# facebookresearch/metamorph

Measured on AMD Instinct MI355X. Metric: train tokens/sec (LLaMA-3-8B + SigLIP-SO400M, seq2048, 256 img toks), whole job, higher is better.
Workload: dtype bf16

## Files before the change

metamorph_amd/build.py:

```python
from __future__ import annotations

import hashlib
import os
import subprocess
import sys

PKG = os.path.dirname(os.path.abspath(__file__))
CSRC = os.path.join(PKG, "csrc")
LIBDIR = os.path.join(PKG, "lib")
LIB = os.path.join(LIBDIR, "libmm355.so")
SOURCES = ["gemm_bf16.hip", "rowwise.hip", "elementwise.hip", "attn.hip", "attn2.hip", "attn4.hip", "attn4_bwd.hip", "decode.hip", "decode_w8.hip", "decode_w4.hip", "decode_kv8.hip", "attn_extend.hip", "gemm_w8.hip", "gemm_w4.hip", "losses.hip", "linear_ce.hip"]
HEADERS = ["mm355_common.h", "gemm_common.h", "splitk.h", "decode_wq.h", "attn2.h", "rowsum.h"] + sorted(
    os.path.join(d, f) for d in ("attn4_gen", "attn4_bwd_gen")
    for f in os.listdir(os.path.join(CSRC, d)) if f.endswith(".inc"))
BASE_FLAGS = ["--offload-arch=gfx950", "-O3", "-std=c++17", "-fPIC", "-Wno-unused-result"]
FLAGS = BASE_FLAGS + ["-mllvm", "-amdgpu-mfma-vgpr-form=1"]
FLAGS_OF = {f: BASE_FLAGS + ["-mllvm", "-amdgpu-spill-vgpr-to-agpr=0"] for f in ("attn4.hip", "attn4_bwd.hip")}


def _hipcc():
    for c in (os.environ.get("HIPCC"), "/opt/rocm/bin/hipcc", "hipcc"):
        if c and (os.path.isabs(c) and os.path.exists(c) or not os.path.isabs(c)):
            return c
    raise RuntimeError("hipcc not found")


def _digest():
    h = hashlib.sha256()
    for f in SOURCES + HEADERS:
        h.update(open(os.path.join(CSRC, f), "rb").read())
    h.update(open(os.path.join(os.path.dirname(PKG), "include", "mm355.h"), "rb").read())
    h.update(" ".join(FLAGS).encode())
    h.update(repr(sorted(FLAGS_OF.items())).encode())
    return h.hexdigest()


def build(force: bool = False, verbose: bool = True) -> str:
    os.makedirs(LIBDIR, exist_ok=True)
    stamp = os.path.join(LIBDIR, "libmm355.stamp")
    dig = _digest()
    if not force and os.path.exists(LIB) and os.path.exists(stamp) and open(stamp).read().strip() == dig:
        return LIB
    hipcc = _hipcc()
    objs = []
    procs = []
    for src in SOURCES:
        obj = os.path.join(LIBDIR, src.replace(".hip", ".o"))
        cmd = [hipcc, *FLAGS_OF.get(src, FLAGS), "-c", os.path.join(CSRC, src), "-o", obj]
        if verbose:
            print("[mm355 build]", " ".join(cmd), flush=True)
        procs.append((src, subprocess.Popen(cmd, stdout=subprocess.PIPE, stderr=subprocess.STDOUT)))
        objs.append(obj)
    for src, p in procs:
        out, _ = p.communicate()
        if p.returncode != 0:
            raise RuntimeError(f"hipcc failed on {src}:\n{out.decode(errors='replace')}")
    cmd = [hipcc, "--offload-arch=gfx950", "-shared", "-fPIC", "-o", LIB, *objs]
    if verbose:
        print("[mm355 build]", " ".join(cmd), flush=True)
    subprocess.check_call(cmd)
    with open(stamp, "w") as f:
        f.write(dig)
    return LIB


# ... 3 lines not shown
```

metamorph_amd/csrc/elementwise.hip:

```cpp
#include "mm355_common.h"
#include <algorithm>

namespace {

constexpr int NT = 256;
constexpr int MAX_GRID = 256 * 16;

inline unsigned grid_for(int64_t work_items) {
    int64_t g = (work_items + NT - 1) / NT;
    if (g > MAX_GRID) g = MAX_GRID;
    if (g < 1) g = 1;
    return (unsigned)g;
}

__global__ void rope_table_kernel(uint16_t* __restrict__ cos_o, uint16_t* __restrict__ sin_o, int L, int d, float theta) {
    const int half = d >> 1;
    for (int64_t i = blockIdx.x * (int64_t)NT + threadIdx.x; i < (int64_t)L * half; i += (int64_t)gridDim.x * NT) {
        const int l = (int)(i / half), j = (int)(i % half);
        const float inv = 1.0f / powf(theta, (float)(2 * j) / (float)d);
        const float ang = (float)l * inv;
        const uint16_t c = f2bf(cosf(ang)), s = f2bf(sinf(ang));
        cos_o[(int64_t)l * d + j] = c; cos_o[(int64_t)l * d + half + j] = c;
        sin_o[(int64_t)l * d + j] = s; sin_o[(int64_t)l * d + half + j] = s;
    }
// ... 125 lines not shown
        float f[8];
        unpack8(*(const u32x4*)(x + i), f);
#pragma unroll
        for (int e = 0; e < 8; ++e) f[e] = kind == MM355_GELU_ERF ? gelu_erf_f(f[e]) : gelu_tanh_f(f[e]);
        *(u32x4*)(y + i) = pack8(f);
    }
}
__global__ __launch_bounds__(NT) void gelu_bwd_kernel(const uint16_t* __restrict__ x, const uint16_t* __restrict__ dy, uint16_t* __restrict__ dx, int64_t n, int kind) {
    for (int64_t i = (blockIdx.x * (int64_t)NT + threadIdx.x) * 8; i < n; i += (int64_t)gridDim.x * NT * 8) {
        float f[8], g[8];
        unpack8(*(const u32x4*)(x + i), f);
        unpack8(*(const u32x4*)(dy + i), g);
#pragma unroll
        for (int e = 0; e < 8; ++e) g[e] *= kind == MM355_GELU_ERF ? gelu_erf_grad(f[e]) : gelu_tanh_grad(f[e]);
        *(u32x4*)(dx + i) = pack8(g);
    }
}

__global__ __launch_bounds__(NT) void scale_kernel(uint16_t* __restrict__ x, int64_t n, const float* __restrict__ s_dev, float s_host) {
    const float s = (s_dev ? *s_dev : 1.0f) * s_host;
    const int64_t nv = n >> 3;
    for (int64_t v = blockIdx.x * (int64_t)NT + threadIdx.x; v < nv; v += (int64_t)gridDim.x * NT) {
        float f[8];
        unpack8(*(const u32x4*)(x + v * 8), f);
#pragma unroll
        for (int e = 0; e < 8; ++e) f[e] *= s;
        *(u32x4*)(x + v * 8) = pack8(f);
    }
    if (blockIdx.x == 0 && threadIdx.x < (n & 7)) { const int64_t i = (nv << 3) + threadIdx.x; x[i] = f2bf(bf2f(x[i]) * s); }
}
template <typename TX>
__global__ __launch_bounds__(NT) void axpy_kernel(uint16_t* __restrict__ y, const TX* __restrict__ x, int64_t n, const float* __restrict__ s_dev,
                                                  float s_host, int accumulate) {
    const float s = (s_dev ? *s_dev : 1.0f) * s_host;
    for (int64_t i = blockIdx.x * (int64_t)NT + threadIdx.x; i < n; i += (int64_t)gridDim.x * NT) {
        float xv;
        if constexpr (sizeof(TX) == 2) xv = bf2f(x[i]); else xv = x[i];
        float r = s * xv;
        if (accumulate) r += bf2f(y[i]);
        y[i] = f2bf(r);
    }
}
__global__ __launch_bounds__(NT) void cast2d_kernel(const float* __restrict__ in, int64_t ld_in, uint16_t* __restrict__ out, int64_t ld_out, int64_t rows, int cols) {
    const int cv = cols >> 3;
    const int64_t total = rows * cv;
    for (int64_t i = blockIdx.x * (int64_t)NT + threadIdx.x; i < total; i += (int64_t)gridDim.x * NT) {
        const int64_t r = i / cv; const int c = (int)(i % cv) * 8;
        const f32x4 a = *(const f32x4*)(in + r * ld_in + c), b = *(const f32x4*)(in + r * ld_in + c + 4);
        const float f[8] = {a.x, a.y, a.z, a.w, b.x, b.y, b.z, b.w};
        *(u32x4*)(out + r * ld_out + c) = pack8(f);
    }
}

__global__ __launch_bounds__(NT) void adamw_kernel(float* __restrict__ p32, float* __restrict__ m, float* __restrict__ v, const uint16_t* __restrict__ g,
                                                   uint16_t* __restrict__ pout, int64_t n, float lr, float b1, float b2, float eps, float wd,
                                                   float bc1, float bc2, const float* __restrict__ gs_dev) {
    const float gs = gs_dev ? *gs_dev : 1.0f;
    const float inv_sqrt_bc2 = rsqrtf(bc2);
    const float step = lr / bc1;
    for (int64_t i = blockIdx.x * (int64_t)NT + threadIdx.x; i < n; i += (int64_t)gridDim.x * NT) {
        const float gr = bf2f(g[i]) * gs;
        float p = p32[i] * (1.0f - lr * wd);
        const float mi = m[i] * b1 + (1.0f - b1) * gr;
        const float vi = v[i] * b2 + (1.0f - b2) * gr * gr;
        const float denom = sqrtf(vi) * inv_sqrt_bc2 + eps;
        p -= step * (mi / denom);
        m[i] = mi; v[i] = vi; p32[i] = p;
        pout[i] = f2bf(p);
    }
}
__global__ __launch_bounds__(NT) void sumsq_kernel(const uint16_t* __restrict__ x, int64_t n, float* __restrict__ partials) {
    __shared__ float red[NT / 64];
    float s = 0.f;
    const int64_t nv = n >> 3;
    for (int64_t v = blockIdx.x * (int64_t)NT + threadIdx.x; v < nv; v += (int64_t)gridDim.x * NT) {
        float f[8];
        unpack8(*(const u32x4*)(x + v * 8), f);
#pragma unroll
        for (int e = 0; e < 8; ++e) s += f[e] * f[e];
    }
    if (blockIdx.x == 0 && threadIdx.x < (n & 7)) { const float f = bf2f(x[(nv << 3) + threadIdx.x]); s += f * f; }
    s = block_sum<NT>(s, red);
    if (threadIdx.x == 0) partials[blockIdx.x] = s;
}
__global__ __launch_bounds__(NT) void sumsq_finish_kernel(const float* __restrict__ partials, int count, float* __restrict__ out) {
    __shared__ float red[NT / 64];
    float s = 0.f;
    for (int i = threadIdx.x; i < count; i += NT) s += partials[i];
    s = block_sum<NT>(s, red);
    if (threadIdx.x == 0) out[0] += s;
}
__global__ void clip_coef_kernel(const float* __restrict__ sumsq, float max_norm, float pre, float* __restrict__ coef) {
    const float nrm = sqrtf(*sumsq);
    float c = max_norm > 0.f ? max_norm / (nrm + 1e-6f) : 1.0f;
    if (c > 1.0f) c = 1.0f;
    *coef = c * pre;
}

template <typename TI>
__global__ __launch_bounds__(NT) void im2col_kernel(const TI* __restrict__ img, int N, int H, int W, int p, uint16_t* __restrict__ out, int Kp) {
    const int gh = H / p, gw = W / p, kreal = 3 * p * p;
    const int64_t total = (int64_t)N * gh * gw * Kp;
    for (int64_t i = blockIdx.x * (int64_t)NT + threadIdx.x; i < total; i += (int64_t)gridDim.x * NT) {
        const int k = (int)(i % Kp);
        const int64_t pr = i / Kp;
        uint16_t val = 0;
        if (k < kreal) {
            const int c = k / (p * p), dy = (k / p) % p, dx = k % p;
            const int px = (int)(pr % gw), py = (int)((pr / gw) % gh); const int64_t n = pr / ((int64_t)gw * gh);
            const TI x = img[((n * 3 + c) * H + (int64_t)py * p + dy) * W + (int64_t)px * p + dx];
            if constexpr (sizeof(TI) == 2) val = x; else val = f2bf(x);
        }
        out[i] = val;
    }
}

__global__ __launch_bounds__(NT) void splice_gather_kernel(const uint16_t* __restrict__ embed, const uint16_t* __restrict__ proj, const int32_t* __restrict__ src,
                                                           uint16_t* __restrict__ out, int64_t rows, int h) {
    const int64_t row = blockIdx.x * (int64_t)(NT / 64) + (threadIdx.x >> 6);
// ... 103 lines not shown
    if (!gu || !dact || !dgu || M <= 0 || I <= 0 || (I & 7)) return MM355_EINVAL;
    LAUNCH(swiglu_bwd_kernel, grid_for(M * (I / 8)), gu, dact, dgu, act, M, (int)I);
}
extern "C" int mm355_swiglu_bwd_t(const mm355_bf16* gu, const mm355_bf16* dact, mm355_bf16* dgu, mm355_bf16* actT, mm355_bf16* dguT,
                                  int64_t M, int64_t I, void* stream) {
    (void)hipGetLastError();
    if (!gu || !dact || !dgu || !actT || !dguT || M <= 0 || I <= 0) return MM355_EINVAL;
    if ((M & 63) || (I & 63)) return MM355_EUNSUPPORTED;
    if (M / 64 > 65535) return MM355_EINVAL;
    hipLaunchKernelGGL(swiglu_bwd_t_kernel, dim3((unsigned)(I / 64), (unsigned)(M / 64)), dim3(256), 0, (hipStream_t)stream, gu, dact, dgu,
                       actT, dguT, M, (int)I);
    return mm_launch_status();
}
extern "C" int mm355_gelu_fwd(const mm355_bf16* x, mm355_bf16* y, int64_t n, int kind, void* stream) {
    (void)hipGetLastError();
    if (!x || !y || n <= 0 || (n & 7)) return MM355_EINVAL;
    LAUNCH(gelu_fwd_kernel, grid_for(n / 8), x, y, n, kind);
}
extern "C" int mm355_gelu_bwd(const mm355_bf16* x, const mm355_bf16* dy, mm355_bf16* dx, int64_t n, int kind, void* stream) {
    (void)hipGetLastError();
    if (!x || !dy || !dx || n <= 0 || (n & 7)) return MM355_EINVAL;
    LAUNCH(gelu_bwd_kernel, grid_for(n / 8), x, dy, dx, n, kind);
}
extern "C" int mm355_scale_bf16(mm355_bf16* x, int64_t n, const float* s_dev, float s_host, void* stream) {
    (void)hipGetLastError();
    if (!x || n <= 0 || !mm_aligned16(x)) return MM355_EINVAL;
    LAUNCH(scale_kernel, grid_for(n / 8 + 1), x, n, s_dev, s_host);
}
extern "C" int mm355_axpy_bf16(mm355_bf16* y, const mm355_bf16* x, int64_t n, const float* s_dev, float s_host, int accumulate, void* stream) {
    (void)hipGetLastError();
    if (!x || !y || n <= 0) return MM355_EINVAL;
    LAUNCH(axpy_kernel<uint16_t>, grid_for(n), y, x, n, s_dev, s_host, accumulate);
}
extern "C" int mm355_axpy_f32_to_bf16(mm355_bf16* y, const float* x, int64_t n, float s_host, int accumulate, void* stream) {
    (void)hipGetLastError();
    if (!x || !y || n <= 0) return MM355_EINVAL;
    LAUNCH(axpy_kernel<float>, grid_for(n), y, x, n, (const float*)nullptr, s_host, accumulate);
}
extern "C" int mm355_axpy_f32_to_bf16_dev(mm355_bf16* y, const float* x, int64_t n, const float* s_dev, float s_host, int accumulate, void* stream) {
    (void)hipGetLastError();
    if (!x || !y || n <= 0) return MM355_EINVAL;
    LAUNCH(axpy_kernel<float>, grid_for(n), y, x, n, s_dev, s_host, accumulate);
}
extern "C" int mm355_cast_f32_bf16_2d(const float* in, int64_t ld_in, mm355_bf16* out, int64_t ld_out, int64_t rows, int64_t cols, void* stream) {
    (void)hipGetLastError();
    if (!in || !out || rows <= 0 || cols <= 0 || (cols & 7) || (ld_in & 3) || (ld_out & 7)) return MM355_EINVAL;
    LAUNCH(cast2d_kernel, grid_for(rows * (cols / 8)), in, ld_in, out, ld_out, rows, (int)cols);
}
extern "C" int mm355_adamw_shard(float* p32, float* m, float* v, const mm355_bf16* g, mm355_bf16* p_out, int64_t n, float lr, float beta1,
                                 float beta2, float eps, float weight_decay, float bias_corr1, float bias_corr2, const float* grad_scale_dev,
                                 void* stream) {
    (void)hipGetLastError();
    if (!p32 || !m || !v || !g || !p_out || n <= 0 || bias_corr1 <= 0.f || bias_corr2 <= 0.f) return MM355_EINVAL;
    LAUNCH(adamw_kernel, grid_for(n), p32, m, v, g, p_out, n, lr, beta1, beta2, eps, weight_decay, bias_corr1, bias_corr2, grad_scale_dev);
}
extern "C" int mm355_sumsq_bf16(const mm355_bf16* x, int64_t n, float* out, float* partials, void* stream) {
    (void)hipGetLastError();
    if (!x || !out || !partials || n <= 0 || !mm_aligned16(x)) return MM355_EINVAL;
    const int blocks = (int)std::min<int64_t>((n / 8 + NT) / NT, MM355_SUMSQ_PARTIALS);
    hipLaunchKernelGGL(sumsq_kernel, dim3(blocks), dim3(NT), 0, (hipStream_t)stream, x, n, partials);
    hipLaunchKernelGGL(sumsq_finish_kernel, dim3(1), dim3(NT), 0, (hipStream_t)stream, (const float*)partials, blocks, out);
    return mm_launch_status();
}
extern "C" int mm355_clip_coef(const float* sumsq, float max_norm, float pre_scale, float* coef, void* stream) {
    (void)hipGetLastError();
    if (!sumsq || !coef) return MM355_EINVAL;
    hipLaunchKernelGGL(clip_coef_kernel, dim3(1), dim3(1), 0, (hipStream_t)stream, sumsq, max_norm, pre_scale, coef);
    return mm_launch_status();
}
extern "C" int mm355_im2col_patch(const void* images, int images_are_f32, int64_t N, int64_t H, int64_t W, int64_t p, mm355_bf16* out, int64_t Kp,
                                  void* stream) {
    (void)hipGetLastError();
    if (!images || !out || N <= 0 || H < p || W < p || p <= 0 || Kp < 3 * p * p) return MM355_EINVAL;
    const int64_t total = N * (H / p) * (W / p) * Kp;
    if (images_are_f32) LAUNCH(im2col_kernel<float>, grid_for(total), (const float*)images, (int)N, (int)H, (int)W, (int)p, out, (int)Kp);
    LAUNCH(im2col_kernel<uint16_t>, grid_for(total), (const uint16_t*)images, (int)N, (int)H, (int)W, (int)p, out, (int)Kp);
}
extern "C" int mm355_splice_gather(const mm355_bf16* embed, const mm355_bf16* proj, const int32_t* src, mm355_bf16* out, int64_t rows, int64_t h,
                                   void* stream) {
    (void)hipGetLastError();
    if (!embed || !src || !out || rows <= 0 || h <= 0 || (h & 7)) return MM355_EINVAL;
    LAUNCH(splice_gather_kernel, (unsigned)((rows + 3) / 4), embed, proj, src, out, rows, (int)h);
}
extern "C" int mm355_rows_gather(const mm355_bf16* in, int64_t ld_in, const int32_t* idx, mm355_bf16* out, int64_t ld_out, int64_t R, int64_t h,
                                 void* stream) {
    (void)hipGetLastError();
    if (!in || !idx || !out || R <= 0 || h <= 0 || (h & 7) || (ld_in & 7) || (ld_out & 7)) return MM355_EINVAL;
    LAUNCH(rows_gather_kernel, (unsigned)((R + 3) / 4), in, ld_in, idx, out, ld_out, R, (int)h);
}
extern "C" int mm355_rows_scatter_add(const mm355_bf16* src, int64_t ld_src, const int32_t* idx, mm355_bf16* dst, int64_t ld_dst, int64_t R,
                                      int64_t h, void* stream) {
    (void)hipGetLastError();
    if (!src || !idx || !dst || R <= 0 || h <= 0 || (h & 7) || (ld_src & 7) || (ld_dst & 7)) return MM355_EINVAL;
    LAUNCH(rows_scatter_add_kernel, (unsigned)((R + 3) / 4), src, ld_src, idx, dst, ld_dst, R, (int)h);
}
extern "C" int mm355_embed_grad(const mm355_bf16* dout, const int32_t* tok, const int32_t* seg_start, const int32_t* pos, int64_t n_seg,
                                mm355_bf16* dembed, int64_t h, int accumulate, void* stream) {
    (void)hipGetLastError();
    if (!dout || !tok || !seg_start || !pos || !dembed || n_seg <= 0 || h <= 0 || (h & 7)) return MM355_EINVAL;
    LAUNCH(embed_grad_kernel, (unsigned)((n_seg + 3) / 4), dout, tok, seg_start, pos, n_seg, dembed, (int)h, accumulate);
}
```

metamorph_amd/csrc/gemm_bf16.hip:

```cpp
#include "gemm_common.h"
#include "splitk.h"
#include <type_traits>
#include <cstdlib>

namespace {

MM_DEV void gemm_epilogue_swiglu(f32x4 (&acc)[8][4], const GemmArgs& a, unsigned char* smem, int m0, int tn, int wm, int wn, int wave, int lane) {
    constexpr int TN = 64;
    const int fr = lane & 15, fq = lane >> 4;
    const int M = a.M, I = (int)a.res_mod;
    float* stg = (float*)smem + wave * (16 * TN);
    const int row_l = lane >> 2, k4 = lane & 3;
    uint16_t* gu = (uint16_t*)a.C;
    uint16_t* act = (uint16_t*)a.res;
    const int ch0 = tn * 128 + wn * 32;
#pragma unroll
    for (int i = 0; i < 8; ++i) {
        __builtin_amdgcn_fence(__ATOMIC_RELEASE, "wavefront");
        __builtin_amdgcn_wave_barrier();
#pragma unroll
        for (int j = 0; j < 4; ++j)
#pragma unroll
            for (int r = 0; r < 4; ++r) stg[(fq * 4 + r) * TN + j * 16 + fr] = acc[i][j][r];
        __builtin_amdgcn_fence(__ATOMIC_RELEASE, "wavefront");
        __builtin_amdgcn_wave_barrier();
        const int grow = m0 + wm * 128 + i * 16 + row_l;
        if (grow < M) {
            float g[8], u[8], o[8];
            const f32x4 g0 = *(const f32x4*)(stg + row_l * TN + k4 * 8), g1 = *(const f32x4*)(stg + row_l * TN + k4 * 8 + 4);
            const f32x4 u0 = *(const f32x4*)(stg + row_l * TN + 32 + k4 * 8), u1 = *(const f32x4*)(stg + row_l * TN + 32 + k4 * 8 + 4);
            g[0] = g0.x; g[1] = g0.y; g[2] = g0.z; g[3] = g0.w; g[4] = g1.x; g[5] = g1.y; g[6] = g1.z; g[7] = g1.w;
            u[0] = u0.x; u[1] = u0.y; u[2] = u0.z; u[3] = u0.w; u[4] = u1.x; u[5] = u1.y; u[6] = u1.z; u[7] = u1.w;
            const u32x4 gp = pack8(g), up = pack8(u);
            const int ch = ch0 + k4 * 8;
            *(u32x4*)(gu + (int64_t)grow * a.ldc + ch) = gp;
            *(u32x4*)(gu + (int64_t)grow * a.ldc + I + ch) = up;
            float gb[8], ub[8];
            unpack8(gp, gb);
            unpack8(up, ub);
#pragma unroll
            for (int e = 0; e < 8; ++e) o[e] = round_bf(gb[e] / (1.0f + __expf(-gb[e]))) * ub[e];
            *(u32x4*)(act + (int64_t)grow * a.ldr + ch) = pack8(o);
        }
    }
}

constexpr int SWB_TROW = 144;
constexpr int SWB_T = 3 * 32 * SWB_TROW;
constexpr int SWB_LDS = 32768 + 8 * SWB_T;
MM_DEV void gemm_epilogue_swiglu_bwd(f32x4 (&acc)[8][4], const GemmArgs& a, unsigned char* smem, int m0, int n0, int wm, int wn, int wave, int lane) {
    constexpr int TN = 64, PF = 4;
    typedef __attribute__((ext_vector_type(4))) short s16x4;
    typedef __attribute__((address_space(3))) s16x4* lds4_t;
    const int fr = lane & 15, fq = lane >> 4;
// ... 640 lines not shown
    return (int64_t)a.ntm * a.ntn;
}

template <int ABL = 0>
int launch_gemm_pp_t(GemmArgs a, hipStream_t s) {
    static std::atomic<uint64_t> lds_ok{0};
    if (mm_ensure_dynamic_lds((const void*)gemm_pp_kernel<ABL>, PP_LDS, lds_ok) != MM355_OK) return MM355_ELAUNCH;
    const int64_t total = pp_prepare(a);
    if (total <= 0 || total > 0x7fffffff) return MM355_EINVAL;
#ifdef MM355_PP_PERSIST
    hipLaunchKernelGGL((gemm_pp_kernel<ABL>), dim3((unsigned)std::min<int64_t>(total, MM355_PP_PERSIST)), dim3(512), PP_LDS, s, a);
#else
    hipLaunchKernelGGL((gemm_pp_kernel<ABL>), dim3((unsigned)total), dim3(512), PP_LDS, s, a);
#endif
    return mm_launch_status();
}

int launch_gemm_pp_pair(GemmArgs a0, GemmArgs a1, hipStream_t s) {
    static std::atomic<uint64_t> lds_ok{0};
    if (mm_ensure_dynamic_lds((const void*)gemm_pp_pair_kernel, PP_LDS, lds_ok) != MM355_OK) return MM355_ELAUNCH;
    const int64_t n0 = pp_prepare(a0), n1 = pp_prepare(a1);
    if (n0 <= 0 || n1 <= 0 || n0 + n1 > 0x7fffffff) return MM355_EINVAL;
    hipLaunchKernelGGL(gemm_pp_pair_kernel, dim3((unsigned)(n0 + n1)), dim3(512), PP_LDS, s, a0, a1, (int)n0);
    return mm_launch_status();
}

bool pp_eligible(const GemmArgs& a) {
    if (a.K < 128 || (a.K & 127)) return false;
    const int64_t ea = (256 * a.lda + a.K) * 2;
    const int64_t eb = (256 * a.ldb + a.K) * 2;
    return ea < 0x7fffffffLL && eb < 0x7fffffffLL;
}

int launch_gemm_pp(GemmArgs a, hipStream_t s) {
    if (!pp_eligible(a)) return launch_gemm<256, 256, 2, 4, true, 1>(a, s);
    return launch_gemm_pp_t(a, s);
}

template <int BM, int BN, int WM, int WN, bool GLDS, int PIPE = 0>
int launch_gemm(GemmArgs a, hipStream_t s) {
    constexpr int STAGE = (BM + BN) * 128;
    constexpr int LDS = 2 * STAGE;
    auto kern = gemm_nt_kernel<BM, BN, WM, WN, GLDS, PIPE>;
    static std::atomic<uint64_t> lds_ok{0};
    if (mm_ensure_dynamic_lds((const void*)kern, LDS, lds_ok) != MM355_OK) return MM355_ELAUNCH;
    a.ntm = (a.M + BM - 1) / BM;
    a.ntn = (a.N + BN - 1) / BN;
    const int64_t total = (int64_t)a.ntm * a.ntn;
    if (total <= 0 || total > 0x7fffffff) return MM355_EINVAL;
    hipLaunchKernelGGL(kern, dim3((unsigned)total), dim3(WM * WN * 64), LDS, s, a);
    return mm_launch_status();
}

__global__ __launch_bounds__(256) void transpose_kernel(const uint16_t* __restrict__ in, int64_t ld_in, int rows, int cols,
                                                        uint16_t* __restrict__ out, int64_t ld_out) {
    __shared__ uint16_t tile[64][64 + 2];
    const int r0 = blockIdx.y * 64, c0 = blockIdx.x * 64;
    const int tid = threadIdx.x;
#pragma unroll
    for (int i = 0; i < 2; ++i) {
        const int v = tid + i * 256, r = v >> 3, c = (v & 7) * 8;
        const int gr = r0 + r, gc = c0 + c;
        uint16_t tmp[8];
        if (gr < rows && gc + 8 <= cols) {
            *(u32x4*)tmp = *(const u32x4*)(in + (int64_t)gr * ld_in + gc);
        } else {
#pragma unroll
            for (int e = 0; e < 8; ++e) tmp[e] = (gr < rows && gc + e < cols) ? in[(int64_t)gr * ld_in + gc + e] : (uint16_t)0;
        }
#pragma unroll
        for (int e = 0; e < 8; ++e) tile[r][c + e] = tmp[e];
    }
    __syncthreads();
#pragma unroll
    for (int i = 0; i < 2; ++i) {
        const int v = tid + i * 256, c = v >> 3, r = (v & 7) * 8;
        const int gc = c0 + c, gr = r0 + r;
        if (gc >= cols) continue;
        uint16_t tmp[8];
#pragma unroll
        for (int e = 0; e < 8; ++e) tmp[e] = tile[r + e][c];
        if (gr + 8 <= rows && ((ld_out & 7) == 0)) {
            *(u32x4*)(out + (int64_t)gc * ld_out + gr) = *(const u32x4*)tmp;
        } else {
            for (int e = 0; e < 8; ++e)
                if (gr + e < rows) out[(int64_t)gc * ld_out + gr + e] = tmp[e];
        }
    }
}

__global__ __launch_bounds__(256) void colsum_kernel(const uint16_t* __restrict__ x, int64_t ld, int M, int N, float* __restrict__ out) {
    __shared__ float part[4][64];
    const int cq = threadIdx.x & 63, rp = threadIdx.x >> 6;
    const int c = blockIdx.x * 64 + cq;
    float s = 0.f;
    if (c < N)
        for (int r = rp; r < M; r += 4) s += bf2f(x[(int64_t)r * ld + c]);
    part[rp][cq] = s;
    __syncthreads();
    if (rp == 0 && c < N) out[c] += (part[0][cq] + part[1][cq]) + (part[2][cq] + part[3][cq]);
}

__global__ __launch_bounds__(1024) void colsum8_kernel(const uint16_t* __restrict__ x, int64_t ld, int M, int N, float* __restrict__ out) {
    __shared__ float part[128][65];
    const int cg = threadIdx.x & 7, rp = threadIdx.x >> 3;
    const int c0 = blockIdx.x * 64 + cg * 8;
    float s[8] = {0.f, 0.f, 0.f, 0.f, 0.f, 0.f, 0.f, 0.f};
    if (c0 < N)
        for (int r = rp; r < M; r += 128) {
            float f[8];
            unpack8(*(const u32x4*)(x + (int64_t)r * ld + c0), f);
#pragma unroll
            for (int e = 0; e < 8; ++e) s[e] += f[e];
        }
#pragma unroll
    for (int e = 0; e < 8; ++e) part[rp][cg * 8 + e] = s[e];
    __syncthreads();
    const int c = blockIdx.x * 64 + threadIdx.x;
    if (threadIdx.x < 64 && c < N) {
        float t = 0.f;
        for (int p = 0; p < 128; ++p) t += part[p][threadIdx.x];
        out[c] += t;
    }
}

}

namespace {
__global__ __launch_bounds__(256) void splitk_reduce_kernel(const float* __restrict__ part, int S, int M, int N, const uint16_t* __restrict__ res,
                                                            int64_t ldr, uint16_t* __restrict__ out, int64_t ldc) {
    const int nv = N >> 3;
    const int64_t total = (int64_t)M * nv, plane = (int64_t)M * N;
    for (int64_t i = blockIdx.x * 256ll + threadIdx.x; i < total; i += (int64_t)gridDim.x * 256) {
        const int m = (int)(i / nv), c = (int)(i % nv) * 8;
        float v[8];
        const float* p = part + (int64_t)m * N + c;
        const f32x4 a0 = *(const f32x4*)p, a1 = *(const f32x4*)(p + 4);
        v[0] = a0.x; v[1] = a0.y; v[2] = a0.z; v[3] = a0.w; v[4] = a1.x; v[5] = a1.y; v[6] = a1.z; v[7] = a1.w;
        for (int s = 1; s < S; ++s) {
// ... 345 lines not shown
        const int64_t t256 = ((M + 255) / 256) * ((N + 255) / 256);
        const int64_t t128 = ((M + 127) / 128) * ((N + 127) / 128);
        if (dma_ok) {
            variant = (t256 >= 200) ? 11 : 2;
            if (variant == 2 && t128 < 224 && M > 64 && t128 * 2 >= 64) variant = 9;
        } else variant = 1;
    }
    if (!dma_ok && variant != 1) return MM355_EUNSUPPORTED;
    switch (variant) {
        case 1: return launch_gemm<128, 128, 2, 2, false>(a, s);
        case 2: return launch_gemm<128, 128, 2, 2, true>(a, s);
        case 7: return launch_gemm<256, 256, 2, 4, true, 1>(a, s);
        case 9: return launch_gemm<64, 128, 1, 4, true>(a, s);
        case 11: return launch_gemm_pp(a, s);
#ifdef MM355_ABLATIONS
        case 91: return launch_gemm_pp_t<1>(a, s);
        case 92: return launch_gemm_pp_t<2>(a, s);
        case 93: return launch_gemm_pp_t<3>(a, s);
#endif
        default: return MM355_EUNSUPPORTED;
    }
}

namespace {
int pair_problem(GemmArgs& a, const mm355_bf16* A, int64_t lda, const mm355_bf16* B, int64_t ldb, void* C, int64_t ldc,
                 int64_t M, int64_t N, int64_t K, uint32_t flags) {
    if (!A || !B || !C || M <= 0 || N <= 0 || K <= 0) return MM355_EINVAL;
    if ((K & 7) || (lda & 7) || (ldb & 7) || !mm_aligned16(A) || !mm_aligned16(B) || !mm_aligned16(C)) return MM355_EINVAL;
    if (M > 0x7fffffff || N > 0x7fffffff || K > 0x7fffffff) return MM355_EINVAL;
    if (flags & ~(MM355_GEMM_ACCUMULATE | MM355_GEMM_OUT_F32)) return MM355_EINVAL;
    a.A = A; a.B = B; a.C = C; a.bias = nullptr; a.res = nullptr;
    a.lda = lda; a.ldb = ldb; a.ldc = ldc; a.ldr = 0; a.res_mod = 0;
    a.M = (int)M; a.N = (int)N; a.K = (int)K; a.flags = flags; a.ntm = a.ntn = 0;
    return pp_eligible(a) ? MM355_OK : MM355_EUNSUPPORTED;
}
}

extern "C" int mm355_gemm_pair_bf16(const mm355_bf16* A0, int64_t lda0, const mm355_bf16* B0, int64_t ldb0, void* C0, int64_t ldc0,
                                    int64_t M0, int64_t N0, int64_t K0, uint32_t flags0,
                                    const mm355_bf16* A1, int64_t lda1, const mm355_bf16* B1, int64_t ldb1, void* C1, int64_t ldc1,
                                    int64_t M1, int64_t N1, int64_t K1, uint32_t flags1, void* stream) {
    (void)hipGetLastError();
    GemmArgs a0, a1;
    int rc = pair_problem(a0, A0, lda0, B0, ldb0, C0, ldc0, M0, N0, K0, flags0);
    if (rc != MM355_OK) return rc;
    rc = pair_problem(a1, A1, lda1, B1, ldb1, C1, ldc1, M1, N1, K1, flags1);
    if (rc != MM355_OK) return rc;
    return launch_gemm_pp_pair(a0, a1, (hipStream_t)stream);
}

extern "C" int mm355_transpose_bf16(const mm355_bf16* in, int64_t ld_in, int64_t rows, int64_t cols, mm355_bf16* out,
                                    int64_t ld_out, void* stream) {
    (void)hipGetLastError();
    if (!in || !out || rows <= 0 || cols <= 0 || (ld_in & 7) || !mm_aligned16(in) || !mm_aligned16(out)) return MM355_EINVAL;
    if (ld_out < rows || rows > 0x7fffffff || cols > 0x7fffffff) return MM355_EINVAL;
    dim3 grid((unsigned)((cols + 63) / 64), (unsigned)((rows + 63) / 64));
    hipLaunchKernelGGL(transpose_kernel, grid, dim3(256), 0, (hipStream_t)stream, in, ld_in, (int)rows, (int)cols, out, ld_out);
    return mm_launch_status();
}

extern "C" int mm355_gemm_swiglu_bf16(const mm355_bf16* X, int64_t ldx, const mm355_bf16* Wgu, int64_t ldw, mm355_bf16* gu, int64_t ld_gu,
                                      mm355_bf16* act, int64_t ld_act, int64_t M, int64_t I, int64_t K, void* stream) {
    (void)hipGetLastError();
    if (!X || !Wgu || !gu || !act || M <= 0 || I <= 0 || K <= 0) return MM355_EINVAL;
    if ((ldx & 7) || (ldw & 7) || (ld_gu & 7) || (ld_act & 7) || !mm_aligned16(X) || !mm_aligned16(Wgu) || !mm_aligned16(gu) || !mm_aligned16(act))
        return MM355_EINVAL;
    if (M > 0x7fffffff || I > 0x3fffffff || K > 0x7fffffff) return MM355_EINVAL;
    if ((I & 127) || K < 128 || (K & 127) || (2 * I * ldw + K) * 2 >= 0x7fffffffLL || (256 * ldx + K) * 2 >= 0x7fffffffLL) return MM355_EUNSUPPORTED;
    GemmArgs a = {};
    a.A = X; a.B = Wgu; a.C = gu; a.bias = nullptr; a.res = act;
    a.lda = ldx; a.ldb = ldw; a.ldc = ld_gu; a.ldr = ld_act; a.res_mod = I;
    a.M = (int)M; a.N = (int)(2 * I); a.K = (int)K; a.flags = 0; a.ntm = a.ntn = 0;
    static std::atomic<uint64_t> lds_ok{0};
    if (mm_ensure_dynamic_lds((const void*)gemm_pp_swiglu_kernel, PP_LDS, lds_ok) != MM355_OK) return MM355_ELAUNCH;
    const int64_t total = pp_prepare(a);
    if (total <= 0 || total > 0x7fffffff) return MM355_EINVAL;
    hipLaunchKernelGGL(gemm_pp_swiglu_kernel, dim3((unsigned)total), dim3(512), PP_LDS, (hipStream_t)stream, a);
    return mm_launch_status();
}

extern "C" int mm355_gemm_rope_bf16(const mm355_bf16* X, int64_t ldx, const mm355_bf16* Wqkv, int64_t ldw, mm355_bf16* qkv, int64_t ld_qkv,
                                    const mm355_bf16* cos_t, const mm355_bf16* sin_t, const int32_t* pos_offset,
                                    int64_t M, int64_t N, int64_t K, int64_t L, int64_t n_rot, void* stream) {
    (void)hipGetLastError();
    if (!X || !Wqkv || !qkv || !cos_t || !sin_t || M <= 0 || N <= 0 || K <= 0 || L <= 0 || n_rot < 0 || n_rot > N) return MM355_EINVAL;
    if ((ldx & 7) || (ldw & 7) || (ld_qkv & 7) || !mm_aligned16(X) || !mm_aligned16(Wqkv) || !mm_aligned16(qkv) || !mm_aligned16(cos_t) || !mm_aligned16(sin_t))
        return MM355_EINVAL;
    if (M > 0x7fffffff || N > 0x7fffffff || K > 0x7fffffff || L > 0x7fffffff) return MM355_EINVAL;
    if ((N & 255) || (n_rot & 127) || K < 128 || (K & 127) || (256 * ldx + K) * 2 >= 0x7fffffffLL || (256 * ldw + K) * 2 >= 0x7fffffffLL) return MM355_EUNSUPPORTED;
    GemmArgs a = {};
    a.A = X; a.B = Wqkv; a.C = qkv; a.bias = (const uint16_t*)pos_offset; a.res = nullptr;
    a.lda = ldx; a.ldb = ldw; a.ldc = ld_qkv; a.ldr = 0; a.res_mod = n_rot;
    a.M = (int)M; a.N = (int)N; a.K = (int)K; a.flags = 0; a.ntm = a.ntn = 0;
    a.aux0 = (uint16_t*)cos_t; a.aux1 = (uint16_t*)sin_t; a.ld_aux = L;
    static std::atomic<uint64_t> lds_ok{0};
    if (mm_ensure_dynamic_lds((const void*)gemm_pp_rope_kernel, PP_LDS, lds_ok) != MM355_OK) return MM355_ELAUNCH;
    const int64_t total = pp_prepare(a);
    if (total <= 0 || total > 0x7fffffff) return MM355_EINVAL;
    hipLaunchKernelGGL(gemm_pp_rope_kernel, dim3((unsigned)total), dim3(512), PP_LDS, (hipStream_t)stream, a);
    return mm_launch_status();
}

extern "C" int mm355_gemm_swiglu_bwd_bf16(const mm355_bf16* dY, int64_t ldy, const mm355_bf16* WdT, int64_t ldw, const mm355_bf16* gu, int64_t ld_gu,
                                          mm355_bf16* dgu, int64_t ld_dgu, mm355_bf16* actT, mm355_bf16* dguT, int64_t ldT,
                                          int64_t M, int64_t I, int64_t K, void* stream) {
    (void)hipGetLastError();
    if (!dY || !WdT || !gu || !dgu || !actT || !dguT || M <= 0 || I <= 0 || K <= 0) return MM355_EINVAL;
    if ((ldy & 7) || (ldw & 7) || (ld_gu & 7) || (ld_dgu & 7) || (ldT & 7) || ldT < M || !mm_aligned16(dY) || !mm_aligned16(WdT) || !mm_aligned16(gu)
// ... 28 lines not shown
```

metamorph_amd/csrc/rowwise.hip:

```cpp
#include "mm355_common.h"
#include "rowsum.h"
#include <type_traits>

namespace {

constexpr int NT = 256;

template <int VPT>
__global__ __launch_bounds__(NT) void rmsnorm_fwd_kernel(const uint16_t* __restrict__ x, const uint16_t* __restrict__ w,
                                                         uint16_t* __restrict__ y, float* __restrict__ rstd_out, int h, float eps) {
    __shared__ float red[NT / 64];
    const int64_t row = blockIdx.x;
    const int nv = h >> 3;
    const uint16_t* xr = x + row * h;
    float xv[VPT][8];
    float ss = 0.f;
#pragma unroll
    for (int i = 0; i < VPT; ++i) {
        const int v = threadIdx.x + i * NT;
        if (v < nv) {
            unpack8(*(const u32x4*)(xr + v * 8), xv[i]);
#pragma unroll
            for (int e = 0; e < 8; ++e) ss += xv[i][e] * xv[i][e];
        }
    }
    ss = block_sum<NT>(ss, red);
    const float rstd = rsqrtf(ss / (float)h + eps);
    if (rstd_out && threadIdx.x == 0) rstd_out[row] = rstd;
#pragma unroll
    for (int i = 0; i < VPT; ++i) {
        const int v = threadIdx.x + i * NT;
        if (v < nv) {
            float wv[8], o[8];
            unpack8(*(const u32x4*)(w + v * 8), wv);
#pragma unroll
            for (int e = 0; e < 8; ++e) o[e] = wv[e] * round_bf(xv[i][e] * rstd);
            *(u32x4*)(y + row * h + v * 8) = pack8(o);
        }
    }
}

__global__ __launch_bounds__(256) void rmsnorm_apply_t_kernel(const uint16_t* __restrict__ x, const uint16_t* __restrict__ w,
                                                              const float* __restrict__ rstd, int M, int h,
                                                              uint16_t* __restrict__ out, int64_t ld_out) {
    __shared__ uint16_t tile[64][64 + 2];
    const int r0 = blockIdx.y * 64, c0 = blockIdx.x * 64;
    const int tid = threadIdx.x;
#pragma unroll
    for (int i = 0; i < 2; ++i) {
        const int v = tid + i * 256, r = v >> 3, c = (v & 7) * 8;
        const int gr = r0 + r, gc = c0 + c;
        uint16_t tmp[8];
        if (gr < M && gc + 8 <= h) {
            float xv[8], wv[8], o[8];
            unpack8(*(const u32x4*)(x + (int64_t)gr * h + gc), xv);
            unpack8(*(const u32x4*)(w + gc), wv);
            const float rs = rstd[gr];
#pragma unroll
            for (int e = 0; e < 8; ++e) o[e] = wv[e] * round_bf(xv[e] * rs);
            *(u32x4*)tmp = pack8(o);
        } else {
#pragma unroll
            for (int e = 0; e < 8; ++e) tmp[e] = 0;
        }
#pragma unroll
        for (int e = 0; e < 8; ++e) tile[r][c + e] = tmp[e];
    }
    __syncthreads();
#pragma unroll
    for (int i = 0; i < 2; ++i) {
        const int v = tid + i * 256, c = v >> 3, r = (v & 7) * 8;
        const int gc = c0 + c, gr = r0 + r;
        if (gc >= h) continue;
        uint16_t tmp[8];
#pragma unroll
        for (int e = 0; e < 8; ++e) tmp[e] = tile[r + e][c];
        if (gr + 8 <= M && ((ld_out & 7) == 0)) {
            *(u32x4*)(out + (int64_t)gc * ld_out + gr) = *(const u32x4*)tmp;
        } else {
            for (int e = 0; e < 8; ++e)
                if (gr + e < M) out[(int64_t)gc * ld_out + gr + e] = tmp[e];
        }
    }
}

template <int VPT>
__global__ __launch_bounds__(NT) void rmsnorm_bwd_kernel(const uint16_t* __restrict__ dy, const uint16_t* __restrict__ x,
                                                         const uint16_t* __restrict__ w, const uint16_t* __restrict__ dres,
                                                         uint16_t* __restrict__ dx, float* __restrict__ dw,
                                                         float* __restrict__ ws, int M, int h, float eps, int rows_per_block) {
    __shared__ float red[NT / 64];
    const int nv = h >> 3;
    float wv[VPT][8], dwacc[VPT][8];
#pragma unroll
    for (int i = 0; i < VPT; ++i) {
        const int v = threadIdx.x + i * NT;
#pragma unroll
        for (int e = 0; e < 8; ++e) { dwacc[i][e] = 0.f; wv[i][e] = 0.f; }
        if (v < nv) unpack8(*(const u32x4*)(w + v * 8), wv[i]);
    }
    const int r0 = blockIdx.x * rows_per_block, r1 = min(M, r0 + rows_per_block);
    for (int row = r0; row < r1; ++row) {
        const uint16_t* xr = x + (int64_t)row * h;
        const uint16_t* gr = dy + (int64_t)row * h;
        float xv[VPT][8], gv[VPT][8];
        float ss = 0.f;
#pragma unroll
        for (int i = 0; i < VPT; ++i) {
            const int v = threadIdx.x + i * NT;
            if (v < nv) {
                unpack8(*(const u32x4*)(xr + v * 8), xv[i]);
                unpack8(*(const u32x4*)(gr + v * 8), gv[i]);
#pragma unroll
                for (int e = 0; e < 8; ++e) ss += xv[i][e] * xv[i][e];
            }
        }
        ss = block_sum<NT>(ss, red);
        const float rstd = rsqrtf(ss / (float)h + eps);
        float dot = 0.f;
#pragma unroll
        for (int i = 0; i < VPT; ++i) {
            const int v = threadIdx.x + i * NT;
            if (v < nv) {
#pragma unroll
                for (int e = 0; e < 8; ++e) {
                    const float xh = xv[i][e] * rstd;
                    dwacc[i][e] += gv[i][e] * round_bf(xh);
                    gv[i][e] *= wv[i][e];
                    dot += gv[i][e] * xh;
                }
            }
        }
        dot = block_sum<NT>(dot, red) / (float)h;
#pragma unroll
// ... 376 lines not shown
        const float nrm = fmaxf(round_bf(sqrtf(ss)), 1e-12f);
        inv = 1.0f / nrm;
        dot *= inv * inv;
    }
    const float w00 = (1.0f - lx) * (1.0f - ly), w01 = lx * (1.0f - ly), w10 = (1.0f - lx) * ly, w11 = lx * ly;
    for (int v = lane; v < nv; v += 64) {
        float r[8], gy[8];
        unpack8(*(const u32x4*)(g + v * 8), gy);
        if (normalize) interp(v, r);
#pragma unroll
        for (int e = 0; e < 8; ++e) {
            const float dr = normalize ? (gy[e] - r[e] * dot) * inv : gy[e];
            if (si == so) atomicAdd(din + o00 + v * 8 + e, dr);
            else {
                atomicAdd(din + o00 + v * 8 + e, dr * w00);
                atomicAdd(din + o01 + v * 8 + e, dr * w01);
                atomicAdd(din + o10 + v * 8 + e, dr * w10);
                atomicAdd(din + o11 + v * 8 + e, dr * w11);
            }
        }
    }
}

template <typename F>
int dispatch_vpt(int h, F&& f) {
    const int nv = h >> 3;
    if (nv <= NT) return f(std::integral_constant<int, 1>{});
    if (nv <= 2 * NT) return f(std::integral_constant<int, 2>{});
    if (nv <= 4 * NT) return f(std::integral_constant<int, 4>{});
    if (nv <= 8 * NT) return f(std::integral_constant<int, 8>{});
    return MM355_EUNSUPPORTED;
}

}

extern "C" int mm355_rmsnorm_fwd_rstd(const mm355_bf16* x, const mm355_bf16* w, mm355_bf16* y, float* rstd_out, int64_t M, int64_t h, float eps,
                                      void* stream) {
    (void)hipGetLastError();
    if (!x || !w || !y || M <= 0 || h <= 0 || (h & 7) || M > 0x7fffffff) return MM355_EINVAL;
    return dispatch_vpt((int)h, [&](auto vpt) {
        hipLaunchKernelGGL((rmsnorm_fwd_kernel<decltype(vpt)::value>), dim3((unsigned)M), dim3(NT), 0, (hipStream_t)stream, x, w, y, rstd_out,
                           (int)h, eps);
        return mm_launch_status();
    });
}
extern "C" int mm355_rmsnorm_fwd(const mm355_bf16* x, const mm355_bf16* w, mm355_bf16* y, int64_t M, int64_t h, float eps, void* stream) {
    return mm355_rmsnorm_fwd_rstd(x, w, y, nullptr, M, h, eps, stream);
}
extern "C" int mm355_rmsnorm_apply_t(const mm355_bf16* x, const mm355_bf16* w, const float* rstd, int64_t M, int64_t h, mm355_bf16* out_t,
                                     int64_t ld_out, void* stream) {
    (void)hipGetLastError();
    if (!x || !w || !rstd || !out_t || M <= 0 || h <= 0 || (h & 7) || M > 0x7fffffff || ld_out < M) return MM355_EINVAL;
    if (!mm_aligned16(x) || !mm_aligned16(w) || !mm_aligned16(out_t)) return MM355_EINVAL;
    dim3 grid((unsigned)((h + 63) / 64), (unsigned)((M + 63) / 64));
    hipLaunchKernelGGL(rmsnorm_apply_t_kernel, grid, dim3(256), 0, (hipStream_t)stream, x, w, rstd, (int)M, (int)h, out_t, ld_out);
    return mm_launch_status();
}

constexpr int DWR_COLS = 32;
__global__ __launch_bounds__(256) void rmsnorm_dw_reduce_kernel(const float* __restrict__ ws, float* __restrict__ dw, int G, int h, int ld) {
    __shared__ f32x4 part[32][8];
    const int cq = threadIdx.x & 7, rl = threadIdx.x >> 3;
    const int c = blockIdx.x * DWR_COLS + cq * 4;
    f32x4 acc0 = {0.f, 0.f, 0.f, 0.f}, acc1 = {0.f, 0.f, 0.f, 0.f};
    if (c < h) {
        const float* p = ws + c;
        int g = rl;
        for (; g + 32 < G; g += 64) {
            acc0 += *(const f32x4*)(p + (int64_t)g * ld);
            acc1 += *(const f32x4*)(p + (int64_t)(g + 32) * ld);
        }
        if (g < G) acc0 += *(const f32x4*)(p + (int64_t)g * ld);
    }
    part[rl][cq] = acc0 + acc1;
    __syncthreads();
    if (rl == 0 && c < h) {
        f32x4 s = part[0][cq];
#pragma unroll
        for (int r = 1; r < 32; ++r) s += part[r][cq];
#pragma unroll
        for (int e = 0; e < 4; ++e) dw[c + e] += s[e];
    }
}

__global__ __launch_bounds__(256) void rmsnorm_dw_reduce_bf16_kernel(const float* __restrict__ ws, uint16_t* __restrict__ grad, int G, int h, int ld,
                                                                     int accumulate) {
    __shared__ f32x4 part[32][8];
    const int cq = threadIdx.x & 7, rl = threadIdx.x >> 3;
    const int c = blockIdx.x * DWR_COLS + cq * 4;
    f32x4 acc0 = {0.f, 0.f, 0.f, 0.f}, acc1 = {0.f, 0.f, 0.f, 0.f};
    if (c < h) {
        const float* p = ws + c;
        int g = rl;
        for (; g + 32 < G; g += 64) {
            acc0 += *(const f32x4*)(p + (int64_t)g * ld);
            acc1 += *(const f32x4*)(p + (int64_t)(g + 32) * ld);
        }
        if (g < G) acc0 += *(const f32x4*)(p + (int64_t)g * ld);
    }
    part[rl][cq] = acc0 + acc1;
    __syncthreads();
    if (rl == 0 && c < h) {
        f32x4 s = part[0][cq];
#pragma unroll
        for (int r = 1; r < 32; ++r) s += part[r][cq];
#pragma unroll
// ... 136 lines not shown
```

Baseline: 26890.

## Vectorize AdamW and add 128x128 swizzled-LDS transpose kernels for large shapes

The AdamW update now processes eight elements per thread with 16-byte vector loads and stores, plus an alignment head and scalar tail, and uses explicit FMA ordering. A new shared header provides 128x128 tile transpose helpers with an XOR-swizzled LDS layout and perm-based 8x8 regrouping. These helpers back new wide variants of the generic bf16 transpose and the fused rmsnorm-apply-transpose, used when the grid reaches at least 2048 tiles. The aim is fewer memory instructions and better coalescing on bandwidth-bound kernels, at the cost of more code paths and slightly changed float rounding order in AdamW.

```diff
diff --git a/metamorph_amd/build.py b/metamorph_amd/build.py
--- a/metamorph_amd/build.py
+++ b/metamorph_amd/build.py
@@ -10,7 +10,7 @@
 LIBDIR = os.path.join(PKG, "lib")
 LIB = os.path.join(LIBDIR, "libmm355.so")
 SOURCES = ["gemm_bf16.hip", "rowwise.hip", "elementwise.hip", "attn.hip", "attn2.hip", "attn4.hip", "attn4_bwd.hip", "decode.hip", "decode_w8.hip", "decode_w4.hip", "decode_kv8.hip", "attn_extend.hip", "gemm_w8.hip", "gemm_w4.hip", "losses.hip", "linear_ce.hip"]
-HEADERS = ["mm355_common.h", "gemm_common.h", "splitk.h", "decode_wq.h", "attn2.h", "rowsum.h"] + sorted(
+HEADERS = ["mm355_common.h", "gemm_common.h", "splitk.h", "decode_wq.h", "attn2.h", "rowsum.h", "transpose_tile.h"] + sorted(
     os.path.join(d, f) for d in ("attn4_gen", "attn4_bwd_gen")
     for f in os.listdir(os.path.join(CSRC, d)) if f.endswith(".inc"))
 BASE_FLAGS = ["--offload-arch=gfx950", "-O3", "-std=c++17", "-fPIC", "-Wno-unused-result"]
diff --git a/metamorph_amd/csrc/elementwise.hip b/metamorph_amd/csrc/elementwise.hip
--- a/metamorph_amd/csrc/elementwise.hip
+++ b/metamorph_amd/csrc/elementwise.hip
@@ -201,19 +201,52 @@
     }
 }
 
+MM_DEV void adamw_elem(float& p, float& mi, float& vi, float gr, float decay, float b1, float b2, float eps, float inv_sqrt_bc2, float step) {
+#pragma clang fp contract(off)
+    vi = vi * b2 + (1.0f - b2) * gr * gr;
+    mi = __builtin_fmaf(1.0f - b1, gr, mi * b1);
+    const float denom = __builtin_fmaf(sqrtf(vi), inv_sqrt_bc2, eps);
+    p = p * decay - step * (mi / denom);
+}
 __global__ __launch_bounds__(NT) void adamw_kernel(float* __restrict__ p32, float* __restrict__ m, float* __restrict__ v, const uint16_t* __restrict__ g,
                                                    uint16_t* __restrict__ pout, int64_t n, float lr, float b1, float b2, float eps, float wd,
-                                                   float bc1, float bc2, const float* __restrict__ gs_dev) {
+                                                   float bc1, float bc2, const float* __restrict__ gs_dev, int head, int64_t nv) {
     const float gs = gs_dev ? *gs_dev : 1.0f;
     const float inv_sqrt_bc2 = rsqrtf(bc2);
     const float step = lr / bc1;
-    for (int64_t i = blockIdx.x * (int64_t)NT + threadIdx.x; i < n; i += (int64_t)gridDim.x * NT) {
-        const float gr = bf2f(g[i]) * gs;
-        float p = p32[i] * (1.0f - lr * wd);
-        const float mi = m[i] * b1 + (1.0f - b1) * gr;
-        const float vi = v[i] * b2 + (1.0f - b2) * gr * gr;
-        const float denom = sqrtf(vi) * inv_sqrt_bc2 + eps;
-        p -= step * (mi / denom);
+    const float decay = __builtin_fmaf(-lr, wd, 1.0f);
+    for (int64_t i = blockIdx.x * (int64_t)NT + threadIdx.x; i < nv; i += (int64_t)gridDim.x * NT) {
+        const int64_t o = head + i * 8;
+        const u32x4 gq = *(const u32x4*)(g + o);
+        f32x4 pq[2], mq[2], vq[2];
+#pragma unroll
+        for (int k = 0; k < 2; ++k) {
+            pq[k] = *(const f32x4*)(p32 + o + 4 * k);
+            mq[k] = *(const f32x4*)(m + o + 4 * k);
+            vq[k] = *(const f32x4*)(v + o + 4 * k);
+        }
+        float gf[8], po[8];
+        unpack8(gq, gf);
+#pragma unroll
+        for (int e = 0; e < 8; ++e) {
+            float p = pq[e >> 2][e & 3], mi = mq[e >> 2][e & 3], vi = vq[e >> 2][e & 3];
+            adamw_elem(p, mi, vi, gf[e] * gs, decay, b1, b2, eps, inv_sqrt_bc2, step);
+            pq[e >> 2][e & 3] = p; mq[e >> 2][e & 3] = mi; vq[e >> 2][e & 3] = vi;
+            po[e] = p;
+        }
+#pragma unroll
+        for (int k = 0; k < 2; ++k) {
+            *(f32x4*)(m + o + 4 * k) = mq[k];
+            *(f32x4*)(v + o + 4 * k) = vq[k];
+            *(f32x4*)(p32 + o + 4 * k) = pq[k];
+        }
+        *(u32x4*)(pout + o) = pack8(po);
+    }
+    const int64_t ns = n - nv * 8;
+    for (int64_t j = blockIdx.x * (int64_t)NT + threadIdx.x; j < ns; j += (int64_t)gridDim.x * NT) {
+        const int64_t i = j < head ? j : j + nv * 8;
+        float p = p32[i], mi = m[i], vi = v[i];
+        adamw_elem(p, mi, vi, bf2f(g[i]) * gs, decay, b1, b2, eps, inv_sqrt_bc2, step);
         m[i] = mi; v[i] = vi; p32[i] = p;
         pout[i] = f2bf(p);
     }
@@ -423,7 +456,15 @@
                                  void* stream) {
     (void)hipGetLastError();
     if (!p32 || !m || !v || !g || !p_out || n <= 0 || bias_corr1 <= 0.f || bias_corr2 <= 0.f) return MM355_EINVAL;
-    LAUNCH(adamw_kernel, grid_for(n), p32, m, v, g, p_out, n, lr, beta1, beta2, eps, weight_decay, bias_corr1, bias_corr2, grad_scale_dev);
+    int head = (int)(((16 - ((uintptr_t)g & 15)) & 15) / 2);
+    int64_t nv = 0;
+    if (!((uintptr_t)g & 1) && n >= head + 8 && mm_aligned16(p32 + head) && mm_aligned16(m + head) && mm_aligned16(v + head) &&
+        mm_aligned16(p_out + head))
+        nv = (n - head) / 8;
+    else
+        head = 0;
+    LAUNCH(adamw_kernel, grid_for(nv > 0 ? nv : n), p32, m, v, g, p_out, n, lr, beta1, beta2, eps, weight_decay, bias_corr1, bias_corr2,
+           grad_scale_dev, head, nv);
 }
 extern "C" int mm355_sumsq_bf16(const mm355_bf16* x, int64_t n, float* out, float* partials, void* stream) {
     (void)hipGetLastError();
diff --git a/metamorph_amd/csrc/gemm_bf16.hip b/metamorph_amd/csrc/gemm_bf16.hip
--- a/metamorph_amd/csrc/gemm_bf16.hip
+++ b/metamorph_amd/csrc/gemm_bf16.hip
@@ -1,5 +1,6 @@
 #include "gemm_common.h"
 #include "splitk.h"
+#include "transpose_tile.h"
 #include <type_traits>
 #include <cstdlib>
 
@@ -746,6 +747,10 @@
     return mm_launch_status();
 }
 
+#ifndef MM355_TRANSPOSE_WIDE_MIN_TILES
+#define MM355_TRANSPOSE_WIDE_MIN_TILES 2048
+#endif
+constexpr int64_t TRANSPOSE_WIDE_MIN_TILES = MM355_TRANSPOSE_WIDE_MIN_TILES;
 __global__ __launch_bounds__(256) void transpose_kernel(const uint16_t* __restrict__ in, int64_t ld_in, int rows, int cols,
                                                         uint16_t* __restrict__ out, int64_t ld_out) {
     __shared__ uint16_t tile[64][64 + 2];
@@ -756,7 +761,7 @@
         const int v = tid + i * 256, r = v >> 3, c = (v & 7) * 8;
         const int gr = r0 + r, gc = c0 + c;
         uint16_t tmp[8];
-        if (gr < rows && gc + 8 <= cols) {
+        if (gr < rows && gc + 8 <= cols && (ld_in & 7) == 0) {
             *(u32x4*)tmp = *(const u32x4*)(in + (int64_t)gr * ld_in + gc);
         } else {
 #pragma unroll
@@ -779,6 +784,59 @@
         } else {
             for (int e = 0; e < 8; ++e)
                 if (gr + e < rows) out[(int64_t)gc * ld_out + gr + e] = tmp[e];
+        }
+    }
+}
+
+template <bool EDGE>
+__global__ __launch_bounds__(256) void transpose_wide_kernel(const uint16_t* __restrict__ in, int64_t ld_in, int rows, int cols,
+                                                             uint16_t* __restrict__ out, int64_t ld_out) {
+    __shared__ __attribute__((aligned(16))) uint8_t tile[TT_LDS_BYTES];
+    const int r0 = blockIdx.y * TT_TILE, c0 = blockIdx.x * TT_TILE;
+    const int tid = threadIdx.x;
+    if constexpr (!EDGE) {
+        u32x4 ldv[TT_LOADS];
+#pragma unroll
+        for (int i = 0; i < TT_LOADS; ++i) {
+            int r, slot;
+            tt_load_pos(tid, i, r, slot);
+            ldv[i] = *(const u32x4*)(in + (int64_t)(r0 + r) * ld_in + c0 + slot * 8);
+        }
+#pragma unroll
+        for (int i = 0; i < TT_LOADS; ++i) {
+            int r, slot;
+            tt_load_pos(tid, i, r, slot);
+            tt_put(tile, r, slot, ldv[i]);
+        }
+    } else {
+#pragma unroll 1
+        for (int i = 0; i < TT_LOADS; ++i) {
+            int r, slot;
+            tt_load_pos(tid, i, r, slot);
+            const int gr = r0 + r, gc = c0 + slot * 8;
+            u32x4 q = u32x4{0u, 0u, 0u, 0u};
+            if (gr < rows && gc + 8 <= cols && (ld_in & 7) == 0) {
+                q = *(const u32x4*)(in + (int64_t)gr * ld_in + gc);
+            } else if (gr < rows) {
+#pragma unroll
+                for (int e = 0; e < 8; ++e)
+                    if (gc + e < cols) q[e >> 1] |= (uint32_t)in[(int64_t)gr * ld_in + gc + e] << (16 * (e & 1));
+            }
+            tt_put(tile, r, slot, q);
+        }
+    }
+    __syncthreads();
+#pragma unroll
+    for (int i = 0; i < TT_ITEMS; ++i) {
+        int rb, cq;
+        tt_item_pos(tid, i, rb, cq);
+        u32x4 o[4];
+        tt_get4(tile, rb, cq, o);
+#pragma unroll
+        for (int j = 0; j < 4; ++j) {
+            const int gc = c0 + cq * 4 + j;
+            if constexpr (!EDGE) *(u32x4*)(out + (int64_t)gc * ld_out + r0 + rb * 8) = o[j];
+            else if (gc < cols) tt_store_run(out, ld_out, gc, r0 + rb * 8, rows, o[j]);
         }
     }
 }
@@ -1230,8 +1288,17 @@
 extern "C" int mm355_transpose_bf16(const mm355_bf16* in, int64_t ld_in, int64_t rows, int64_t cols, mm355_bf16* out,
                                     int64_t ld_out, void* stream) {
     (void)hipGetLastError();
-    if (!in || !out || rows <= 0 || cols <= 0 || (ld_in & 7) || !mm_aligned16(in) || !mm_aligned16(out)) return MM355_EINVAL;
+    if (!in || !out || rows <= 0 || cols <= 0 || !mm_aligned16(in) || !mm_aligned16(out)) return MM355_EINVAL;
     if (ld_out < rows || rows > 0x7fffffff || cols > 0x7fffffff) return MM355_EINVAL;
+    const int64_t wide_x = (cols + TT_TILE - 1) / TT_TILE, wide_y = (rows + TT_TILE - 1) / TT_TILE;
+    if (rows >= TT_TILE && cols >= TT_TILE && wide_x * wide_y >= TRANSPOSE_WIDE_MIN_TILES) {
+        const dim3 wide((unsigned)wide_x, (unsigned)wide_y);
+        if (rows % TT_TILE == 0 && cols % TT_TILE == 0 && (ld_in & 7) == 0 && (ld_out & 7) == 0)
+            hipLaunchKernelGGL(transpose_wide_kernel<false>, wide, dim3(256), 0, (hipStream_t)stream, in, ld_in, (int)rows, (int)cols, out, ld_out);
+        else
+            hipLaunchKernelGGL(transpose_wide_kernel<true>, wide, dim3(256), 0, (hipStream_t)stream, in, ld_in, (int)rows, (int)cols, out, ld_out);
+        return mm_launch_status();
+    }
     dim3 grid((unsigned)((cols + 63) / 64), (unsigned)((rows + 63) / 64));
     hipLaunchKernelGGL(transpose_kernel, grid, dim3(256), 0, (hipStream_t)stream, in, ld_in, (int)rows, (int)cols, out, ld_out);
     return mm_launch_status();
diff --git a/metamorph_amd/csrc/rowwise.hip b/metamorph_amd/csrc/rowwise.hip
--- a/metamorph_amd/csrc/rowwise.hip
+++ b/metamorph_amd/csrc/rowwise.hip
@@ -1,5 +1,6 @@
 #include "mm355_common.h"
 #include "rowsum.h"
+#include "transpose_tile.h"
 #include <type_traits>
 
 namespace {
@@ -80,6 +81,75 @@
         } else {
             for (int e = 0; e < 8; ++e)
                 if (gr + e < M) out[(int64_t)gc * ld_out + gr + e] = tmp[e];
+        }
+    }
+}
+
+#ifndef MM355_APPLY_T_WIDE_MIN_TILES
+#define MM355_APPLY_T_WIDE_MIN_TILES 2048
+#endif
+constexpr int64_t APPLY_T_WIDE_MIN_TILES = MM355_APPLY_T_WIDE_MIN_TILES;
+template <bool EDGE>
+__global__ __launch_bounds__(256) void rmsnorm_apply_t_wide_kernel(const uint16_t* __restrict__ x, const uint16_t* __restrict__ w,
+                                                                   const float* __restrict__ rstd, int M, int h,
+                                                                   uint16_t* __restrict__ out, int64_t ld_out) {
+    __shared__ __attribute__((aligned(16))) uint8_t tile[TT_LDS_BYTES];
+    const int r0 = blockIdx.y * TT_TILE, c0 = blockIdx.x * TT_TILE;
+    const int tid = threadIdx.x;
+    const int gc = c0 + (tid & 15) * 8;
+    const bool col_in = !EDGE || gc + 8 <= h;
+    float wv[8];
+    unpack8(col_in ? *(const u32x4*)(w + gc) : u32x4{0u, 0u, 0u, 0u}, wv);
+    if constexpr (!EDGE) {
+        u32x4 xq[TT_LOADS];
+        float rs[TT_LOADS];
+#pragma unroll
+        for (int i = 0; i < TT_LOADS; ++i) {
+            int r, slot;
+            tt_load_pos(tid, i, r, slot);
+            xq[i] = *(const u32x4*)(x + (int64_t)(r0 + r) * h + gc);
+            rs[i] = rstd[r0 + r];
+        }
+#pragma unroll
+        for (int i = 0; i < TT_LOADS; ++i) {
+            int r, slot;
+            tt_load_pos(tid, i, r, slot);
+            float xv[8], o[8];
+            unpack8(xq[i], xv);
+#pragma unroll
+            for (int e = 0; e < 8; ++e) o[e] = wv[e] * round_bf(xv[e] * rs[i]);
+            tt_put(tile, r, slot, pack8(o));
+        }
+    } else {
+#pragma unroll 1
+        for (int i = 0; i < TT_LOADS; ++i) {
+            int r, slot;
+            tt_load_pos(tid, i, r, slot);
+            const int gr = r0 + r;
+            u32x4 y = u32x4{0u, 0u, 0u, 0u};
+            if (gr < M && col_in) {
+                float xv[8], o[8];
+                unpack8(*(const u32x4*)(x + (int64_t)gr * h + gc), xv);
+                const float rs = rstd[gr];
+#pragma unroll
+                for (int e = 0; e < 8; ++e) o[e] = wv[e] * round_bf(xv[e] * rs);
+                y = pack8(o);
+            }
+            tt_put(tile, r, slot, y);
+        }
+    }
+    __syncthreads();
+#pragma unroll
+    for (int i = 0; i < TT_ITEMS; ++i) {
+        int rb, cq;
+        tt_item_pos(tid, i, rb, cq);
+        u32x4 o[4];
+        tt_get4(tile, rb, cq, o);
+#pragma unroll
+        for (int j = 0; j < 4; ++j) {
+            const int oc = c0 + cq * 4 + j;
+            if constexpr (!EDGE) *(u32x4*)(out + (int64_t)oc * ld_out + r0 + rb * 8) = o[j];
+            else if (oc < h) tt_store_run(out, ld_out, oc, r0 + rb * 8, M, o[j]);
         }
     }
 }
@@ -562,6 +632,15 @@
     (void)hipGetLastError();
     if (!x || !w || !rstd || !out_t || M <= 0 || h <= 0 || (h & 7) || M > 0x7fffffff || ld_out < M) return MM355_EINVAL;
     if (!mm_aligned16(x) || !mm_aligned16(w) || !mm_aligned16(out_t)) return MM355_EINVAL;
+    const int64_t wide_x = (h + TT_TILE - 1) / TT_TILE, wide_y = (M + TT_TILE - 1) / TT_TILE;
+    if (M >= TT_TILE && h >= TT_TILE && wide_x * wide_y >= APPLY_T_WIDE_MIN_TILES) {
+        const dim3 wide((unsigned)wide_x, (unsigned)wide_y);
+        if (M % TT_TILE == 0 && h % TT_TILE == 0 && (ld_out & 7) == 0)
+            hipLaunchKernelGGL(rmsnorm_apply_t_wide_kernel<false>, wide, dim3(256), 0, (hipStream_t)stream, x, w, rstd, (int)M, (int)h, out_t, ld_out);
+        else
+            hipLaunchKernelGGL(rmsnorm_apply_t_wide_kernel<true>, wide, dim3(256), 0, (hipStream_t)stream, x, w, rstd, (int)M, (int)h, out_t, ld_out);
+        return mm_launch_status();
+    }
     dim3 grid((unsigned)((h + 63) / 64), (unsigned)((M + 63) / 64));
     hipLaunchKernelGGL(rmsnorm_apply_t_kernel, grid, dim3(256), 0, (hipStream_t)stream, x, w, rstd, (int)M, (int)h, out_t, ld_out);
     return mm_launch_status();
diff --git a/metamorph_amd/csrc/transpose_tile.h b/metamorph_amd/csrc/transpose_tile.h
--- /dev/null
+++ b/metamorph_amd/csrc/transpose_tile.h
@@ -0,0 +1,37 @@
+#pragma once
+
+#include "mm355_common.h"
+
+constexpr int TT_TILE = 128;
+constexpr int TT_LDS_BYTES = TT_TILE * TT_TILE * 2;
+constexpr int TT_LOADS = 8;
+constexpr int TT_ITEMS = 2;
+
+MM_DEV void tt_load_pos(int tid, int i, int& r, int& slot) { const int v = tid + i * 256; r = v >> 4; slot = v & 15; }
+MM_DEV void tt_put(uint8_t* lds, int r, int slot, const u32x4& v) {
+    *(u32x4*)(lds + r * 256 + ((slot ^ ((r >> 3) & 15)) << 4)) = v;
+}
+MM_DEV void tt_item_pos(int tid, int i, int& rb, int& cq) { const int v = tid + i * 256; rb = v & 15; cq = v >> 4; }
+MM_DEV void tt_get4(const uint8_t* lds, int rb, int cq, u32x4 (&o)[4]) {
+    const uint8_t* p = lds + rb * 8 * 256 + (((cq >> 1) ^ rb) << 4) + (cq & 1) * 8;
+    u32x2 w[8];
+#pragma unroll
+    for (int e = 0; e < 8; ++e) w[e] = *(const u32x2*)(p + e * 256);
+#pragma unroll
+    for (int k = 0; k < 4; ++k) {
+        o[0][k] = __builtin_amdgcn_perm(w[2 * k + 1].x, w[2 * k].x, 0x05040100u);
+        o[1][k] = __builtin_amdgcn_perm(w[2 * k + 1].x, w[2 * k].x, 0x07060302u);
+        o[2][k] = __builtin_amdgcn_perm(w[2 * k + 1].y, w[2 * k].y, 0x05040100u);
+        o[3][k] = __builtin_amdgcn_perm(w[2 * k + 1].y, w[2 * k].y, 0x07060302u);
+    }
+}
+MM_DEV void tt_store_run(uint16_t* __restrict__ out, int64_t ld_out, int64_t orow, int ocol, int n_out, const u32x4& v) {
+    uint16_t* dst = out + orow * ld_out + ocol;
+    if (ocol + 8 <= n_out && ((ld_out & 7) == 0)) {
+        *(u32x4*)dst = v;
+    } else {
+#pragma unroll
+        for (int e = 0; e < 8; ++e)
+            if (ocol + e < n_out) dst[e] = (uint16_t)(v[e >> 1] >> (16 * (e & 1)));
+    }
+}
```

Result: no change. 26910 (median of 3 runs) (+0.1%).
